# jinlinyi/PerspectiveFields

Measured on AMD Instinct MI355X. Metric: images/sec (640x640, Paramnet-360Cities), higher is better.
Workload: dtype f32 (operands fp32 in HBM; contractions as 2-way fp16 split on the MFMA, fp32 accumulate, fp32-class accuracy); 1 GPU; BASELINE configs[2]: batch 32/GPU 640x640 Paramnet-360Cities-edina-centered, fields + ParamNet, 320x320 network inputs resident in HBM (4 distinct synthetic images tiled over the batch; the network is data independent), post-process to 640x640; global_batch=32, parallelism=dp1 (images sharded, all-gather of ParamNet scalars), weights=seeded synthetic checkpoint (no network for the trained .pth), precision=fp32, tiles=shipped tile table + static heuristic (no tuning), gathered_param_rows=32

## Files before the change

include/pf_hip.h:

```cpp
#ifndef PF_HIP_H
#define PF_HIP_H

#include <stddef.h>
#include <stdint.h>

#ifdef __cplusplus
extern "C" {
#endif

typedef struct pf_engine* pf_handle;

enum pf_status {
  PF_OK = 0,
  PF_ERR_ARG = -1,
  PF_ERR_DEVICE = -2,
  PF_ERR_WEIGHTS = -3,
  PF_ERR_WORKSPACE = -4
};

enum pf_arch {
  PF_ARCH_PARAMNET_CENTERED = 0,
  PF_ARCH_PERSNET_CLS = 1,
  PF_ARCH_PARAMNET_UNCENTERED = 2
};
// ... 79 lines not shown
#define PF_DISPATCH_RB_LAUNCHES 2
#define PF_DISPATCH_SPLITK_LAUNCHES 3
#define PF_DISPATCH_SPLITK_MAX_FACTOR 4
#define PF_DISPATCH_WINO_LAUNCHES 5
#define PF_DISPATCH_WINO_HALF_LAUNCHES 6
#define PF_DISPATCH_THIN128_LAUNCHES 7
#define PF_DISPATCH_ATTN64_LAUNCHES 8
#define PF_DISPATCH_MIT_MLP_FUSED_LAUNCHES 9
#define PF_DISPATCH_LN_KERNEL_LAUNCHES 10
#define PF_DISPATCH_CONV_LAUNCHES 11
#define PF_DISPATCH_SB_TENSORS 12
#define PF_DISPATCH_FORKS 13
#define PF_DISPATCH_FORK_ALLOC_CONFLICTS 14
#define PF_DISPATCH_REAL_PEAK_BYTES 15
#define PF_DISPATCH_DRY_PEAK_BYTES 16
#define PF_DISPATCH_COLS 17
int pf_last_dispatch(pf_handle h, int64_t* out, int n);

int pf_postprocess_batch(pf_handle h, int batch, const float* d_pred_gravity, const float* d_pred_latitude, const int32_t* h_hw,
                         float* const* h_up_out, float* const* h_lat_out, void* d_workspace, size_t workspace_bytes, void* stream);

int pf_fields_from_params(int device, const float* d_cam5, int H, int W, float* d_up, float* d_lat, void* stream);

#define PF_FIT_COL_ROLL 0
#define PF_FIT_COL_PITCH 1
#define PF_FIT_COL_VFOV 2
#define PF_FIT_COL_REL_FOCAL 3
#define PF_FIT_COL_GENERAL_VFOV 4
#define PF_FIT_COL_REL_CX 5
#define PF_FIT_COL_REL_CY 6
#define PF_FIT_COL_RMS_UP 7
// ... 118 lines not shown
```

perspectivefields_amd/build.py:

```python
from __future__ import annotations

import hashlib
import os
import shutil
import subprocess
import sys

HERE = os.path.dirname(os.path.abspath(__file__))
CSRC = os.path.join(HERE, "csrc")
ASAN = os.environ.get("PF_ASAN", "0") == "1"
_VARIANT = ("_tune" if os.environ.get("PF_TUNING_BUILD", "0") == "1" else "") + ("_asan" if ASAN else "") + os.environ.get("PF_LIB_SUFFIX", "")
LIBDIR = os.path.join(HERE, "lib" + _VARIANT)
LIB = os.path.join(LIBDIR, "libpf_hip.so")
SOURCES = ["igemm.hip", "igemm_sb.hip", "igemm_sbf.hip", "igemm_sbh.hip", "wino.hip", "attn.hip", "attn_block.hip", "stem7.hip", "thin_linear.hip", "elem.hip", "dw7.hip", "dw7_pk.hip", "cnx_mlp.hip", "mit_mlp.hip", "rb_gemm.hip", "rb_chain.hip", "fit_camera.hip", "fit_camera_usm.hip", "pano_crop.hip", "field_err.hip", "engine.hip", "engine_ops.hip"]
NO_PK_F32_FLAGS = ["-Xclang", "-target-feature", "-Xclang", "-packed-fp32-ops"]
EXTRA_FLAGS = {"dw7.hip": ["-fno-slp-vectorize"], "dw7_pk.hip": ["-fno-slp-vectorize"],
               "attn_block.hip": NO_PK_F32_FLAGS, "stem7.hip": NO_PK_F32_FLAGS, "thin_linear.hip": NO_PK_F32_FLAGS, "cnx_mlp.hip": NO_PK_F32_FLAGS, "mit_mlp.hip": NO_PK_F32_FLAGS, "rb_gemm.hip": NO_PK_F32_FLAGS, "rb_chain.hip": NO_PK_F32_FLAGS, "fit_camera.hip": NO_PK_F32_FLAGS, "fit_camera_usm.hip": NO_PK_F32_FLAGS, "pano_crop.hip": NO_PK_F32_FLAGS, "field_err.hip": NO_PK_F32_FLAGS}
FLAGS = ["--offload-arch=gfx950", "-O3", "-std=c++17", "-fPIC", "-Wall", "-Wno-unused-function", "-fno-gpu-rdc"]
if os.environ.get("PF_TUNING_BUILD", "0") == "1":
    FLAGS.append("-DPF_TUNING_BUILD")
ASAN_HOST_FLAGS = ["-Xarch_host", "-fsanitize=address,undefined", "-Xarch_host", "-fno-omit-frame-pointer", "-Xarch_host", "-fno-sanitize-recover=undefined"]
if ASAN:
    FLAGS = FLAGS + ASAN_HOST_FLAGS


def asan_runtime() -> str:
    clang = os.path.join(os.path.dirname(os.path.realpath(_hipcc())), "..", "lib", "llvm", "bin", "clang")
    if not os.path.exists(clang):
        clang = "/opt/rocm/lib/llvm/bin/clang"
    return subprocess.run([clang, "-print-file-name=libclang_rt.asan-x86_64.so"], capture_output=True, text=True, check=True).stdout.strip()


# ... 66 lines not shown
```

perspectivefields_amd/csrc/engine.hip:

```cpp
#include <hip/hip_runtime.h>

#include <algorithm>
#include <cmath>
#include <cstdarg>
#include <cstdio>
#include <cstdlib>
#include <cstring>
#include <map>
#include <string>
#include <unordered_map>
#include <vector>

#include "../../include/pf_hip.h"
#include "pf_kernels.h"

using namespace pf;

namespace {

}
namespace pf_host { thread_local std::string g_create_error; }
#include "host_pack.h"
using namespace pf_host;
namespace {
// ... 34 lines not shown
};
struct LNW { float* g = nullptr; float* b = nullptr; int C = 0; float eps = 1e-6f; };
struct DwW { float* w = nullptr; float* b = nullptr; int C = 0; float in_limit = 65504.f;  };

struct RbLin { unsigned short* w = nullptr; size_t bytes = 0; float* inv = nullptr; float* b = nullptr; int N = 0, K = 0; float sat_limit = 65504.f; };
struct RbSrKv { unsigned short* w = nullptr; size_t bytes = 0; float *sr_inv = nullptr, *sr_b = nullptr, *kv_inv = nullptr, *kv_b = nullptr; };
struct RbProjFc1 { unsigned short* w = nullptr; size_t bytes = 0; };
struct MitBlock { LNW n1, n2, srn; RbLin rq, rkv, rproj, rfc1, rfc2; RbSrKv rsrkv; RbProjFc1 rpf; ConvW qln ; ConvW q, kv, proj, sr, fc1, fc2; DwW dw; unsigned short* mlp_w = nullptr; float* mlp_tab = nullptr;
                  unsigned short* a64_w = nullptr; float* a64_tab = nullptr;
                  unsigned short* tq_w = nullptr; float* tq_tab = nullptr; unsigned short* tp_w = nullptr; float* tp_tab = nullptr;  };
struct MitStage { ConvW pe; LNW pen, norm; std::vector<MitBlock> blocks; };
struct Head {
  ConvW lin[4], proc[4], fold[4], r1c1[4], r1c2[4], r2c1[4], r2c2[4], conv0, conv1, predcls;
  float* predw = nullptr; float* predb = nullptr; int nout = 0;
};
struct CnxBlock { float out_limit = 65504.f;  DwW dw; LNW n; ConvW pw1, pw2; unsigned short* mlp_w = nullptr; float* mlp_tab = nullptr;  };
struct Cnx { ConvW stem, ds[3]; LNW stemn, dsn[3], norm; std::vector<CnxBlock> blocks[4]; float* headw = nullptr; float* headb = nullptr; int nout = 0; };

struct SbT {
  unsigned short* p = nullptr;
  size_t plane = 0;
};
struct Ten {
  float* f = nullptr;
  SbT s;
  Ten() {}
  Ten(float* f_) : f(f_) {}
  Ten(float* f_, SbT s_) : f(f_), s(s_) {}
};

struct Profiler;
// ... 207 lines not shown
  int splitk_mode = -1;
  int wino_half = 1;
  bool can_fork(const Ctx& c) { return side_stream_mode && !c.dry && !c.tuning && (!c.prof || c.prof->min_work > 0.0) && side_ready(); }
  bool sba_heads = false;
  int rb_chain = 60;
  int rb_min_blocks = 192;
  int num_cus = 256;
  int wino_min_hw = 20;
  int wino_min_blocks = 96;
  int wino_tile = -1;
  unsigned* d_sat = nullptr;
  float static_window_max = 0.f;
  int mit_mlp128 = 4;
  bool fuse_mit_mlp = true;
  bool fuse_cnx_mlp = true;
  bool fold_mlp = true;
  int nterms = NT_F16X3;
  DebugSink dbg;
  DebugSink* debug_sink = nullptr;
  struct GraphEntry { std::vector<uintptr_t> key; hipGraphExec_t exec; };
  std::vector<GraphEntry> graphs;
  bool sba = false;

  MitStage stages[4];
  ConvW ll;
  Head heads[2];
  Cnx cnx;
  bool has_param = false;
  int param_in = NET;
  float mean3[3] = {103.53f, 116.28f, 123.675f};
// ... 389 lines not shown
          cb.dw = make_dw(b + ".dwconv", C, 7);
          cb.n = make_ln(b + ".norm", C, 1e-6f);
          cb.pw1 = make_linear(b + ".pwconv1", 4 * C, C, nullptr, b + ".norm", 1e-6f);
          const std::vector<float>& gm = get(b + ".gamma", {C}).data;
          std::vector<double> sc(gm.begin(), gm.end());
          cb.pw2 = make_linear(b + ".pwconv2", C, 4 * C, sc.data());
          if (fuse_cnx_mlp && cnx_mlp_preferred(C)) {
            std::vector<unsigned short> wpk;
            std::vector<float> tab;
            cnx_mlp_pack(get(b + ".pwconv1.weight", {4 * C, C}).data.data(), get(b + ".pwconv1.bias", {4 * C}).data.data(), get(b + ".norm.weight", {C}).data.data(),
                         get(b + ".norm.bias", {C}).data.data(), get(b + ".pwconv2.weight", {C, 4 * C}).data.data(), get(b + ".pwconv2.bias", {C}).data.data(), gm.data(), C,
                         &wpk, &tab);
            cb.mlp_w = upload_u16(wpk);
            cb.mlp_tab = upload(tab);
          }
          cnx.blocks[s].push_back(cb);
        }
      }
      for (int s = 0; s < 4; ++s) {
        if (s > 0) cnx.ds[s - 1].sat_limit = cnx.blocks[s][0].dw.in_limit;
        for (size_t j = 0; j < cnx.blocks[s].size(); ++j) {
          const float lim = j + 1 < cnx.blocks[s].size() ? cnx.blocks[s][j + 1].dw.in_limit : 65504.f;
          cnx.blocks[s][j].out_limit = lim;
          cnx.blocks[s][j].pw2.sat_limit = lim;
        }
      }
      note_static(ln_bound(p + "downsample_layers.0.1", CNX_DIMS[0]), cnx.blocks[0][0].dw.in_limit);
      for (int s = 0; s < 4; ++s)
        for (int j = 0; j < CNX_DEPTHS[s]; ++j) {
          const std::string b = p + "stages." + std::to_string(s) + "." + std::to_string(j);
          if (cnx.blocks[s][j].mlp_w) note_static(mlp_hidden_bound(b + ".norm", b + ".pwconv1", "", CNX_DIMS[s]), 65504.f);
        }
      cnx.norm = make_ln(p + "norm", CNX_DIMS[3], 1e-6f);
      cnx.headw = upload(get(p + "head.weight", {cnx.nout, CNX_DIMS[3]}).data);
      cnx.headb = upload(get(p + "head.bias", {cnx.nout}).data);
    }
    for (auto& kv : host)
      if (!kv.second.used) throw fmt("unexpected checkpoint tensor '%s' for this architecture", kv.first.c_str());
    host.clear();
  }

  void tap(Ctx& c, const std::string& name, const float* p, int B, int H, int W, int C) {
    DebugSink* d = c.dbg;
    if (!d || !d->shadow || !p) return;
    const size_t bytes = (size_t)B * H * W * C * 4, off = (d->used + 255) & ~(size_t)255;
    d->taps.push_back({name, off, {B, H, W, C}});
// ... 512 lines not shown
      if (s > 0) {
        const long Mi = (long)B * h * h;
        const Ten yn_in = S ? Ten(nullptr, c.alloc_sb(Mi * CNX_DIMS[s - 1])) : Ten(y);
        ln(c, cnx.dsn[s - 1], y, yn_in, Mi);
        float* yn = c.alloc((size_t)B * (h / 2) * (h / 2) * C);
        conv(c, cnx.ds[s - 1], yn_in, B, h, h, Ten(yn));
        y = yn;
        h /= 2;
      }
      const long M = (long)B * h * h;
      const size_t mk = c.mark();
      float* d = c.alloc(M * C);
      const Ten dn = S ? Ten(nullptr, c.alloc_sb(M * C)) : Ten(d);
      const Ten hb = c.ten(M * 4 * C, !S, S);
      int blk = -1;
      for (CnxBlock& cb : cnx.blocks[s]) {
        if (blk >= 0) tap(c, fmt("pn.s%d.b%d", s + 1, blk), y, B, h, h, C);
        ++blk;
        if (!c.dry) {
          ProfScope ps(c.prof, c.s, PC_DW7, 8.0 * M * C);
          launch_dwconv7x7(y, cb.dw.w, cb.dw.b, d, B, h, h, C, c.s);
        }
        if (cb.mlp_w && nterms == NT_F16X3) {
          range_in(c, fmt("cnx_mlp s%d.b%d d (LN-fused)", s + 1, blk), d, (size_t)M * C);
          if (!c.dry) {
            ProfScope ps(c.prof, c.s, PC_IGEMM_SB, 2.0 * 2.0 * M * (double)C * 4 * C, (int)M, C, 8 * C, 1);
            launch_cnx_mlp(d, y, cb.mlp_w, cb.mlp_tab, M, C, cb.n.eps, c.s, d_sat, cb.out_limit);
          }
          continue;
        }
        if (cb.pw1.ln_s) {
          gemm(c, cb.pw1, Ten(d), M, hb, ACT_GELU);
        } else {
          ln(c, cb.n, d, dn, M);
          gemm(c, cb.pw1, dn, M, hb, ACT_GELU);
        }
        gemm(c, cb.pw2, hb, M, Ten(y), ACT_NONE, y);
      }
      if (blk >= 0) tap(c, fmt("pn.s%d.b%d", s + 1, blk), y, B, h, h, C);
      c.release(mk);
    }
    float* raw = c.alloc((size_t)B * 8);
// ... 172 lines not shown
  if (const char* v = getenv("PF_WINO")) e->wino_min_hw = atoi(v);
  if (const char* v = getenv("PF_WINO_MIN_BLOCKS")) e->wino_min_blocks = atoi(v);
  {
    const char* wt = getenv("PF_WINO_TILE");
    for (int t = 0; t < conv_num_tiles(); ++t) if (strcmp(conv_tile_name(t), wt ? wt : "wino256x64d") == 0) e->wino_tile = t;
  }
  if (const char* v = getenv("PF_RB_CHAIN")) e->rb_chain = atoi(v);
  if (const char* v = getenv("PF_DEFER_AT")) e->defer_at = atoi(v);
  if (const char* v = getenv("PF_DEFER_PRIO")) e->defer_prio = atoi(v);
  if (!host_only) {
    hipDeviceProp_t prop;
    if (hipGetDeviceProperties(&prop, device) == hipSuccess && prop.multiProcessorCount > 0) e->num_cus = prop.multiProcessorCount;
    e->rb_min_blocks = e->num_cus * 3 / 4;
  }
  if (const char* v = getenv("PF_RB_MIN_BLOCKS")) e->rb_min_blocks = atoi(v);
#ifdef PF_TUNING_BUILD
#endif
  if (const char* v = getenv("PF_SIDE_STREAM")) e->side_stream_mode = atoi(v);
  if (const char* v = getenv("PF_S3_SPLIT")) e->s3_split = atoi(v);
  if (const char* v = getenv("PF_ATTN64")) e->attn64 = atoi(v);
  if (const char* v = getenv("PF_STEM7")) e->stem7 = atoi(v);
  if (const char* v = getenv("PF_THIN128")) e->thin128 = atoi(v);
  if (const char* v = getenv("PF_SBA_HEADS")) e->sba_heads = atoi(v) != 0;
  if (const char* v = getenv("PF_AUTOTUNE")) e->autotune = atoi(v) != 0;
  if (const char* v = getenv("PF_SPLIT_BF16")) e->split_bf16 = atoi(v) != 0;
  if (const char* v = getenv("PF_SBA")) e->sba = atoi(v) != 0;
  e->splitk_mode = conv_splitk_env();
  e->wino_half = conv_wino_half_env();
  if (!e->split_bf16) e->sba = false;
  if (!e->split_bf16 || e->sba) e->fuse_ln = false;
  if (!e->split_bf16 || e->sba) e->fuse_cnx_mlp = false;
  if (!e->split_bf16 || e->sba) e->fuse_mit_mlp = false;

  tune_cache_load(e);
  *out = e;
  return PF_OK;
}

int pf_set_precision(pf_handle h, int mode) {
  if (!h) return PF_ERR_ARG;
  if (mode != PF_PRECISION_FP32 && mode != PF_PRECISION_FP32_BF16X6) return h->fail(PF_ERR_ARG, "pf_set_precision: unknown mode (0 = FP32 split-f16, 3 = FP32_BF16X6; the reduced-precision modes 1 / 2 of earlier versions are gone)");
  if (mode != PF_PRECISION_FP32 && !h->split_bf16) return h->fail(PF_ERR_ARG, "pf_set_precision: this mode needs the split kernels (PF_SPLIT_BF16=0 is set)");
  if (h->pn_pending) { h->issue_deferred(); (void)hipStreamSynchronize(h->pstream); h->pn_pending = false; }
  h->ws_cache.clear();
  h->nterms = mode == PF_PRECISION_FP32_BF16X6 ? 6 : NT_F16X3;
  return PF_OK;
}
// ... 649 lines not shown
```

perspectivefields_amd/csrc/engine_ops.hip:

```cpp
#include "host_pack.h"

using namespace pf;
using namespace pf_host;

extern "C" {

int pf_op_num_conv_tiles(void) { return conv_num_tiles(); }
const char* pf_op_conv_tile_name(int id) { return conv_tile_name(id); }

int pf_op_conv2d(int device, const float* x, const float* x2, int B, int H, int W, int C1, int C2, const float* hw, const float* hb,
                 int Cout, int KH, int KW, int stride, int pad, int act, const float* res1, const float* res2, int post_relu,
                 int nchw_out, int tile_id, float* y, const uint16_t* x_planes, long x_plane_elems, const uint16_t* x2_planes,
                 long x2_plane_elems, uint16_t* y_planes, long y_plane_elems, int precision_flags, void* stream) {
  const int precision = precision_flags & 15;
  const bool allow_splitk = !(precision_flags & 16);
  if (precision != PF_PRECISION_FP32 && precision != PF_PRECISION_FP32_BF16X6) { g_create_error = "pf_op_conv2d: precision must be 0 (split-f16) or 3 (exact bf16 split)"; return PF_ERR_ARG; }
  std::string err;
  int rc = check_device(device, &err);
  if (rc != PF_OK) { g_create_error = err; return rc; }
  const int Cin = C1 + C2;
  if (Cin % 4 != 0 || (C2 > 0 && C1 % 32 != 0)) { g_create_error = "pf_op_conv2d: Cin must be a multiple of 4 (pad on the host), C1 of 32 when concatenating"; return PF_ERR_ARG; }
  hipStream_t s = static_cast<hipStream_t>(stream);
  TmpDev tmp;
  ConvParams p;
// ... 331 lines not shown
    float t = 0.f;
    (void)hipEventElapsedTime(&t, a, b);
    *ms_out = t / iters;
    (void)hipEventDestroy(a); (void)hipEventDestroy(b);
  }
  rc = hipGetLastError() == hipSuccess ? PF_OK : PF_ERR_DEVICE;
  tmp.sync_free(s);
  return rc;
}

int pf_op_cnx_mlp(int device, const float* d, float* y, long rows, int C, const float* w1, const float* b1, const float* lng, const float* lnb, float eps,
                  const float* w2, const float* b2, const float* ls, int iters, float* ms_out, void* stream) {
  std::string err;
  int rc = check_device(device, &err);
  if (rc != PF_OK) { g_create_error = err; return rc; }
  if (!cnx_mlp_supported(C) || !d || !y || rows <= 0) { g_create_error = "pf_op_cnx_mlp: C must be 96 or 192"; return PF_ERR_ARG; }
  hipStream_t s = static_cast<hipStream_t>(stream);
  TmpDev tmp;
  std::vector<unsigned short> wpk;
  std::vector<float> tab;
  cnx_mlp_pack(w1, b1, lng, lnb, w2, b2, ls, C, &wpk, &tab);
  const unsigned short* dw = tmp.up_u16(wpk);
  const float* dt = tmp.up(tab);
  launch_cnx_mlp(d, y, dw, dt, rows, C, eps, s);
  if (iters > 0 && ms_out) {
    hipEvent_t a, b;
    (void)hipEventCreate(&a); (void)hipEventCreate(&b);
    (void)hipEventRecord(a, s);
    for (int i = 0; i < iters; ++i) launch_cnx_mlp(d, y, dw, dt, rows, C, eps, s);
    (void)hipEventRecord(b, s);
    (void)hipEventSynchronize(b);
    float t = 0.f;
    (void)hipEventElapsedTime(&t, a, b);
    *ms_out = t / iters;
    (void)hipEventDestroy(a); (void)hipEventDestroy(b);
  }
  rc = hipGetLastError() == hipSuccess ? PF_OK : PF_ERR_DEVICE;
  tmp.sync_free(s);
  return rc;
}

int pf_op_conv2d_bench(int device, int B, int H, int W, int Cin, int Cout, int K, int stride, int pad, int tile_id, int iters, int fmt_prec, float* ms_out) {
  const int fmt = fmt_prec & 15, precision = fmt_prec >> 4;
  std::string err;
// ... 286 lines not shown
```

perspectivefields_amd/csrc/host_pack.h:

```cpp
#pragma once
#include <hip/hip_runtime.h>

#include <algorithm>
#include <cmath>
#include <cstdarg>
#include <cstdio>
#include <cstdlib>
#include <cstring>
#include <string>
#include <vector>

#include "../../include/pf_hip.h"
#include "pf_kernels.h"

namespace pf_host {
using namespace pf;

extern thread_local std::string g_create_error;

inline int roundup(int v, int m) { return (v + m - 1) / m * m; }

inline std::string fmt(const char* f, ...) {
  char buf[1024];
  va_list ap;
// ... 130 lines not shown
  const int npass = N / cols, nct = cols / 32, steps = K / 16;
  const size_t step_us = (size_t)nct * 2 * 512;
  stream->assign(((size_t)npass * steps + 4) * step_us, 0);
  for (int ps = 0; ps < npass; ++ps)
    for (int st = 0; st < steps; ++st) {
      unsigned short* o = stream->data() + ((size_t)ps * steps + st) * step_us;
      for (int ct = 0; ct < nct; ++ct)
        for (int p = 0; p < 2; ++p)
          for (int lane = 0; lane < 64; ++lane)
            for (int e = 0; e < 8; ++e)
              o[((size_t)(ct * 2 + p) * 64 + lane) * 8 + e] = pl.planes[p * n_all + (size_t)(ps * cols + 32 * ct + (lane & 31)) * K + 16 * st + 8 * (lane >> 5) + e];
    }
  *inv = pl.inv_scale;
}

inline void mit_mlp_pack(const float* w1, const float* b1, const float* g, const float* be, const float* wdw , const float* bdw, const float* w2, const float* b2,
                  int C, std::vector<unsigned short>* wpk, std::vector<float>* tab2) {
  const int H = 4 * C, S1 = C / 16, Q = C / 32, NCH = H / 32;
  std::vector<float> w1f, b1f, cs1;
  fold_ln_linear(w1, b1, g, be, H, C, &w1f, &b1f, &cs1);
  std::vector<float> w2v(w2, w2 + (size_t)C * H);
  const F16Planes p1 = split_f16x2(w1f, H), p2 = split_f16x2(w2v, C);
  const size_t n1 = w1f.size(), n2 = w2v.size();
  const size_t chunk_us = (size_t)mit_mlp_chunk_bytes(C) / 2, w1_us = (size_t)S1 * 2 * 512, w2_us = (size_t)Q * 2 * 2 * 512;
  wpk->assign((size_t)NCH * chunk_us, 0);
  for (int t = 0; t < NCH; ++t) {
    unsigned short* o = wpk->data() + (size_t)t * chunk_us;
    for (int s = 0; s < S1; ++s)
      for (int pl = 0; pl < 2; ++pl)
        for (int lane = 0; lane < 64; ++lane)
// ... 57 lines not shown
```

perspectivefields_amd/csrc/pf_kernels.h:

```cpp
#pragma once
#include <vector>
#include <hip/hip_runtime.h>
#include <stddef.h>
#include <stdint.h>

namespace pf {

enum Act { ACT_NONE = 0, ACT_RELU = 1, ACT_GELU = 2 };
#if defined(__HIPCC__)
__device__ __forceinline__ void sat_watch4(unsigned* sat, float limit, float a, float b, float c, float d) {
  const float mx = fmaxf(fmaxf(fabsf(a), fabsf(b)), fmaxf(fabsf(c), fabsf(d)));
  const float s = (a + b) + (c + d);
  if (!(mx <= limit) || s != s) atomicAdd(sat, 1u);
}
__device__ __forceinline__ float sat_acc4(float amax, float a, float b, float c, float d) {
  return __builtin_fmaxf(__builtin_fmaxf(__builtin_fmaxf(amax, __builtin_fabsf(a)), __builtin_fabsf(b)), __builtin_fmaxf(__builtin_fabsf(c), __builtin_fabsf(d)));
}
__device__ __forceinline__ void sat_flush(unsigned* sat, float limit, float amax) {
  if (sat && amax > limit) atomicAdd(sat, 1u);
}
#endif
#if defined(__HIP_DEVICE_COMPILE__)
#define PF_NO_PK_F32 __attribute__((target("no-packed-fp32-ops")))
#else
// ... 189 lines not shown
  int n;
  int H[MAX], W[MAX];
  float rh[MAX], rw[MAX], sxs[MAX], sys[MAX];
  const float* g2[MAX];
  const float* l1[MAX];
  float* up[MAX];
  float* lat[MAX];
};
void launch_postprocess_batch(PostBatch& pb, int h, int w, int lat_is_sin, hipStream_t s);

void launch_nearest_nhwc4(const float* x, float* y, int B, int H, int W, int Ho, int Wo, hipStream_t s);

bool cnx_mlp_supported(int C);
bool cnx_mlp_preferred(int C);
void launch_cnx_mlp(const float* d, float* y, const unsigned short* wpk, const float* tab, long M, int C, float eps, hipStream_t s, unsigned* sat = nullptr, float sat_limit = 65504.f);
bool mit_mlp_supported(int C);
bool mit_mlp_preferred(int C, int with128);
int mit_mlp_chunk_bytes(int C);
void launch_mit_mlp(const float* x, float* y, const unsigned short* wpk, const float* tab2, int B, int Hs, int Ws, int C, float eps, hipStream_t s, unsigned* sat = nullptr, float sat_limit = 65504.f);
struct RbLinArgs {
  const float* x;
  const float* ln_g;
  const float* ln_b;
  float ln_eps;
  const unsigned short* w;
  size_t w_bytes;
  const float* inv;
  const float* bias;
  const float* res;
  float* y;
// ... 115 lines not shown
```

perspectivefields_amd/csrc/rb_common.h:

```cpp
#pragma once
#include "igemm_common.h"
#include "sb_split.h"

namespace pf {

static constexpr int RB_ROWS = 64;
static constexpr int RB_D = 4;

typedef _Float16 rb_f16x8 __attribute__((ext_vector_type(8)));
__device__ __forceinline__ f32x16 rb_mfma(const u32x4 a, const u32x4 b, const f32x16 c) {
  return __builtin_amdgcn_mfma_f32_32x32x16_f16(__builtin_bit_cast(rb_f16x8, a), __builtin_bit_cast(rb_f16x8, b), c, 0, 0, 0);
}

template <int CTW_, bool EXTRA_, int RT_ = 2>
struct RbGeo {
  static constexpr int CTW = CTW_;
  static constexpr bool EXTRA = EXTRA_;
  static constexpr int RT = RT_;
  static constexpr int NW = CTW + (EXTRA ? 1 : 0);
  static constexpr int NACC = RT * CTW + (EXTRA ? 1 : 0);
  static constexpr int NCT = 4 * CTW + (EXTRA ? 2 : 0);
  static constexpr int COLS = NCT * 32;
  static constexpr int STEP_BYTES = NCT * 2048;
  static constexpr int CHS = RT * 2048 + 64;
};

template <class G>
struct RbW {
  __amdgpu_buffer_rsrc_t rw;
  unsigned voff;
  unsigned toff[G::NW];
  u32x4 f[RB_D][G::NW][2];
  __device__ __forceinline__ void init(const unsigned short* w, size_t bytes, int wave, int lane) {
    rw = __builtin_amdgcn_make_buffer_rsrc(const_cast<unsigned short*>(w), 0, (int)(bytes < 0x7fffffffUL ? bytes : 0x7fffffffUL), 0x00020000);
    voff = (unsigned)lane * 16u;
#pragma unroll
    for (int ci = 0; ci < G::NW; ++ci) toff[ci] = (unsigned)__builtin_amdgcn_readfirstlane((ci < G::CTW ? wave + 4 * ci : 4 * G::CTW + (wave >> 1)) * 2048);
  }
  __device__ __forceinline__ void load_frag(int d, int ci, int pl) { f[d][ci][pl] = __builtin_amdgcn_raw_buffer_load_b128(rw, voff + (unsigned)pl * 1024u, toff[ci], 0); }
  __device__ __forceinline__ void advance() { voff += (unsigned)G::STEP_BYTES; }
  __device__ __forceinline__ void load(int d) {
#pragma unroll
    for (int ci = 0; ci < G::NW; ++ci)
#pragma unroll
      for (int pl = 0; pl < 2; ++pl) load_frag(d, ci, pl);
    advance();
  }
  __device__ __forceinline__ void prologue() {
#pragma unroll
    for (int d = 0; d < RB_D; ++d) load(d);
  }
};

template <class G>
struct RbA {
  u32x4 a[G::RT][2];
  u32x4 x[2];
  __device__ __forceinline__ void read(const unsigned char* chunk, int lane, int xr) {
#pragma unroll
    for (int rt = 0; rt < G::RT; ++rt)
#pragma unroll
      for (int pl = 0; pl < 2; ++pl) a[rt][pl] = *reinterpret_cast<const u32x4*>(chunk + (rt * 2 + pl) * 1024 + lane * 16);
    if constexpr (G::EXTRA && G::RT == 2) {
#pragma unroll
      for (int pl = 0; pl < 2; ++pl) x[pl] = *reinterpret_cast<const u32x4*>(chunk + (xr * 2 + pl) * 1024 + lane * 16);
// ... 32 lines not shown
        for (int t = 0; t < 3; ++t)
#pragma unroll
          for (int rt = 0; rt < G::RT; ++rt) acc[G::RT * ci + rt] = rb_mfma(W.f[d][ci][t == 1], A.a[rt][t == 0], acc[G::RT * ci + rt]);
      } else {
#pragma unroll
        for (int t = 0; t < 3; ++t) acc[G::RT * G::CTW] = rb_mfma(W.f[d][ci][t == 1], A.xa(t == 0), acc[G::RT * G::CTW]);
      }
    } else {
      asm volatile("" :: "v"(W.f[d][ci][0]), "v"(W.f[d][ci][1]), "v"(A.a[0][0]), "v"(A.a[G::RT - 1][1]));
    }
    if constexpr ((ABL & 1) == 0) { W.load_frag(d, ci, 0); W.load_frag(d, ci, 1); }
    RB_FENCE();
  }
  W.advance();
}
template <class G, int ABL = 0>
__device__ __forceinline__ void rb_step(f32x16 (&acc)[G::NACC], RbW<G>& W, int d, const RbA<G>& A, RbA<G>& An, const unsigned char* next_chunk, int lane, int xr) {
  if constexpr (ABL != 0) { rb_step_abl<G, ABL>(acc, W, d, A, An, next_chunk, lane, xr); return; }
  constexpr int X = G::CTW, XA = G::RT * G::CTW, RT = G::RT;
  An.read(next_chunk, lane, xr);
  RB_FENCE();
#pragma unroll
  for (int ci = 0; ci < G::CTW; ++ci) {
    const u32x4 (&w)[2] = W.f[d][ci];
#pragma unroll
    for (int rt = 0; rt < RT; ++rt) acc[RT * ci + rt] = rb_mfma(w[0], A.a[rt][1], acc[RT * ci + rt]);
    if (G::EXTRA && ci == 0) {
      acc[XA] = rb_mfma(W.f[d][X][0], A.xa(1), acc[XA]);
      RB_FENCE();
    }
#pragma unroll
    for (int rt = 0; rt < RT; ++rt) acc[RT * ci + rt] = rb_mfma(w[1], A.a[rt][0], acc[RT * ci + rt]);
// ... 40 lines not shown
```

perspectivefields_amd/engine.py:

```python
from __future__ import annotations

import ctypes
import os
from typing import Dict, Optional, Tuple

import numpy as np

from .build import LIB as LIB_PATH

_HERE = os.path.dirname(os.path.abspath(__file__))
TILE_TABLE = os.path.join(_HERE, "tuned", "gfx950_tiles.txt")
NET = 320
PARAMS_STRIDE = 8

PF_OK = 0
DISPATCH_COLUMNS = ("batch", "s3_split_taken", "rb_launches", "splitk_launches", "splitk_max_factor", "wino_launches", "wino_half_launches", "thin128_launches",
                    "attn64_launches", "mit_mlp_fused_launches", "ln_kernel_launches", "conv_launches", "sb_tensors", "forks", "fork_alloc_conflicts",
                    "real_peak_bytes", "dry_peak_bytes")
_STATUS = {0: "PF_OK", -1: "PF_ERR_ARG", -2: "PF_ERR_DEVICE", -3: "PF_ERR_WEIGHTS", -4: "PF_ERR_WORKSPACE"}

_c = ctypes
_P = _c.c_void_p
_SIGNATURES = {
    "pf_version": (_c.c_char_p, []),
    "pf_last_error": (_c.c_char_p, [_P]),
    "pf_create": (_c.c_int, [_c.POINTER(_P), _c.c_int, _c.c_int]),
    "pf_destroy": (_c.c_int, [_P]),
    "pf_load_tensor": (_c.c_int, [_P, _c.c_char_p, _P, _c.POINTER(_c.c_int64), _c.c_int]),
    "pf_finalize_weights": (_c.c_int, [_P]),
    "pf_output_info": (_c.c_int, [_P, _c.POINTER(_c.c_int), _c.POINTER(_c.c_int), _c.POINTER(_c.c_int)]),
    "pf_max_batch": (_c.c_int, []),
    "pf_workspace_bytes": (_c.c_size_t, [_P, _c.c_int]),
    "pf_last_dispatch": (_c.c_int, [_P, _c.POINTER(_c.c_int64), _c.c_int]),
# ... 497 lines not shown
```

Before: 1704 images/sec.

## Fuse ConvNeXt LN+MLP+residual into one row-block kernel for C=384/768

Adds a row-block kernel for ConvNeXt stages 3 and 4 (C=384/768). It fuses LayerNorm, pwconv1, GELU, pwconv2 with layer scale, and the residual add into a single launch. The 4C hidden activation is streamed through LDS in 128-wide chunks instead of being written to HBM, and weights are pre-packed into a fused stream. It is gated by CU-count-based minimum block counts, so small batches fall back to the old path. The cost is a kernel running one block per CU with heavy register and LDS use, and packing complexity.

```diff
diff --git a/include/pf_hip.h b/include/pf_hip.h
--- a/include/pf_hip.h
+++ b/include/pf_hip.h
@@ -117,7 +117,8 @@
 #define PF_DISPATCH_FORK_ALLOC_CONFLICTS 14
 #define PF_DISPATCH_REAL_PEAK_BYTES 15
 #define PF_DISPATCH_DRY_PEAK_BYTES 16
-#define PF_DISPATCH_COLS 17
+#define PF_DISPATCH_CNX_RB_LAUNCHES 17
+#define PF_DISPATCH_COLS 18
 int pf_last_dispatch(pf_handle h, int64_t* out, int n);
 
 int pf_postprocess_batch(pf_handle h, int batch, const float* d_pred_gravity, const float* d_pred_latitude, const int32_t* h_hw,
diff --git a/perspectivefields_amd/build.py b/perspectivefields_amd/build.py
--- a/perspectivefields_amd/build.py
+++ b/perspectivefields_amd/build.py
@@ -12,10 +12,10 @@
 _VARIANT = ("_tune" if os.environ.get("PF_TUNING_BUILD", "0") == "1" else "") + ("_asan" if ASAN else "") + os.environ.get("PF_LIB_SUFFIX", "")
 LIBDIR = os.path.join(HERE, "lib" + _VARIANT)
 LIB = os.path.join(LIBDIR, "libpf_hip.so")
-SOURCES = ["igemm.hip", "igemm_sb.hip", "igemm_sbf.hip", "igemm_sbh.hip", "wino.hip", "attn.hip", "attn_block.hip", "stem7.hip", "thin_linear.hip", "elem.hip", "dw7.hip", "dw7_pk.hip", "cnx_mlp.hip", "mit_mlp.hip", "rb_gemm.hip", "rb_chain.hip", "fit_camera.hip", "fit_camera_usm.hip", "pano_crop.hip", "field_err.hip", "engine.hip", "engine_ops.hip"]
+SOURCES = ["igemm.hip", "igemm_sb.hip", "igemm_sbf.hip", "igemm_sbh.hip", "wino.hip", "attn.hip", "attn_block.hip", "stem7.hip", "thin_linear.hip", "elem.hip", "dw7.hip", "dw7_pk.hip", "cnx_mlp.hip", "mit_mlp.hip", "rb_gemm.hip", "rb_chain.hip", "cnx_rb.hip", "fit_camera.hip", "fit_camera_usm.hip", "pano_crop.hip", "field_err.hip", "engine.hip", "engine_ops.hip"]
 NO_PK_F32_FLAGS = ["-Xclang", "-target-feature", "-Xclang", "-packed-fp32-ops"]
 EXTRA_FLAGS = {"dw7.hip": ["-fno-slp-vectorize"], "dw7_pk.hip": ["-fno-slp-vectorize"],
-               "attn_block.hip": NO_PK_F32_FLAGS, "stem7.hip": NO_PK_F32_FLAGS, "thin_linear.hip": NO_PK_F32_FLAGS, "cnx_mlp.hip": NO_PK_F32_FLAGS, "mit_mlp.hip": NO_PK_F32_FLAGS, "rb_gemm.hip": NO_PK_F32_FLAGS, "rb_chain.hip": NO_PK_F32_FLAGS, "fit_camera.hip": NO_PK_F32_FLAGS, "fit_camera_usm.hip": NO_PK_F32_FLAGS, "pano_crop.hip": NO_PK_F32_FLAGS, "field_err.hip": NO_PK_F32_FLAGS}
+               "attn_block.hip": NO_PK_F32_FLAGS, "stem7.hip": NO_PK_F32_FLAGS, "thin_linear.hip": NO_PK_F32_FLAGS, "cnx_mlp.hip": NO_PK_F32_FLAGS, "mit_mlp.hip": NO_PK_F32_FLAGS, "rb_gemm.hip": NO_PK_F32_FLAGS, "rb_chain.hip": NO_PK_F32_FLAGS, "cnx_rb.hip": NO_PK_F32_FLAGS, "fit_camera.hip": NO_PK_F32_FLAGS, "fit_camera_usm.hip": NO_PK_F32_FLAGS, "pano_crop.hip": NO_PK_F32_FLAGS, "field_err.hip": NO_PK_F32_FLAGS}
 FLAGS = ["--offload-arch=gfx950", "-O3", "-std=c++17", "-fPIC", "-Wall", "-Wno-unused-function", "-fno-gpu-rdc"]
 if os.environ.get("PF_TUNING_BUILD", "0") == "1":
     FLAGS.append("-DPF_TUNING_BUILD")
diff --git a/perspectivefields_amd/csrc/cnx_rb.hip b/perspectivefields_amd/csrc/cnx_rb.hip
--- /dev/null
+++ b/perspectivefields_amd/csrc/cnx_rb.hip
@@ -0,0 +1,205 @@
+#include <stdlib.h>
+
+#include "rb_common.h"
+
+namespace pf {
+
+template <int C>
+__global__ __launch_bounds__(256, 1) void cnx_rb_kernel(const CnxRbArgs p) {
+  static_assert(C == 384 || C == 768, "geometry: 64 x 384 or 32 x 768 row blocks");
+  constexpr int RT = C == 384 ? 2 : 1, ROWS = 32 * RT;
+  using G1 = RbGeo<1, false, RT>;
+  using G2 = RbGeo<C / 128, false, RT>;
+  constexpr int H = 4 * C, HC = G1::COLS, NCH = H / HC, KC = C / 16, KC2 = HC / 16;
+  constexpr int CHS = G1::CHS;
+  constexpr int TPR = 256 / ROWS;
+  constexpr int CPT = KC / TPR;
+  constexpr int TAB = 2 * H + 2 * C, TAB4 = TAB / 4, NTL = (TAB4 + 255) / 256;
+  constexpr int D1 = C == 384 ? 2 * RB_D : RB_D;
+  constexpr unsigned W1_BYTES = KC * G1::STEP_BYTES, W2_BYTES = KC2 * G2::STEP_BYTES;
+  static_assert(HC == 128 && G2::COLS == C && G2::CHS == CHS && KC % TPR == 0 && KC % D1 == 0 && D1 % 2 == 0 && KC2 == 2 * RB_D, "geometry");
+  static_assert(KC2 * CHS >= 4 * 4096, "the epilogue's scratch lives in the A2 region");
+  static_assert(G1::RT == G2::RT && !G1::EXTRA && !G2::EXTRA && sizeof(RbA<G1>) == sizeof(RbA<G2>),
+                "GEMM 2's last look-ahead is handed to GEMM 1 register by register: RbA<G1> and RbA<G2> must be the same fragments");
+  __shared__ __attribute__((aligned(16))) unsigned char As1[KC * CHS];
+  __shared__ __attribute__((aligned(16))) unsigned char As2[KC2 * CHS];
+  __shared__ __attribute__((aligned(16))) float tabs[TAB];
+  const int tid = threadIdx.x, lane = tid & 63, wave = __builtin_amdgcn_readfirstlane(tid >> 6);
+  const int l31 = lane & 31, hi = lane >> 5;
+  const int m0 = blockIdx.x * ROWS;
+  const int nrows = min(ROWS, p.M - m0);
+
+  RbW<G1, D1> W1;
+  RbW<G2> W2;
+  W1.init(p.w, p.w_bytes, wave, lane);
+  W2.init(p.w, p.w_bytes, wave, lane);
+  W2.voff += W1_BYTES;
+
+  {
+    const int r = tid / TPR, q = tid % TPR;
+    const float* xr = p.d + (size_t)(m0 + min(r, nrows - 1)) * C;
+    float4 v[CPT][4];
+#pragma unroll
+    for (int i = 0; i < CPT; ++i)
+#pragma unroll
+      for (int e = 0; e < 4; ++e) v[i][e] = *reinterpret_cast<const float4*>(xr + 16 * (q + TPR * i) + 4 * e);
+    float4 tv[NTL];
+#pragma unroll
+    for (int j = 0; j < NTL; ++j) tv[j] = reinterpret_cast<const float4*>(p.tab)[min(tid + 256 * j, TAB4 - 1)];
+    W1.prologue();
+    float s = 0.f;
+#pragma unroll
+    for (int i = 0; i < CPT; ++i)
+#pragma unroll
+      for (int e = 0; e < 4; ++e) s += (v[i][e].x + v[i][e].y) + (v[i][e].z + v[i][e].w);
+#pragma unroll
+    for (int o = 1; o < TPR; o *= 2) s += __shfl_xor(s, o);
+    const float mu0 = s / (float)C;
+    float s1 = 0.f;
+#pragma unroll
+    for (int i = 0; i < CPT; ++i)
+#pragma unroll
+      for (int e = 0; e < 4; ++e) {
+        v[i][e] = make_float4(v[i][e].x - mu0, v[i][e].y - mu0, v[i][e].z - mu0, v[i][e].w - mu0);
+        s1 += (v[i][e].x + v[i][e].y) + (v[i][e].z + v[i][e].w);
+      }
+#pragma unroll
+    for (int o = 1; o < TPR; o *= 2) s1 += __shfl_xor(s1, o);
+    const float mu = s1 / (float)C;
+    float ss = 0.f;
+#pragma unroll
+    for (int i = 0; i < CPT; ++i)
+#pragma unroll
+      for (int e = 0; e < 4; ++e) {
+        v[i][e] = make_float4(v[i][e].x - mu, v[i][e].y - mu, v[i][e].z - mu, v[i][e].w - mu);
+        ss = fmaf(v[i][e].x, v[i][e].x, fmaf(v[i][e].y, v[i][e].y, fmaf(v[i][e].z, v[i][e].z, fmaf(v[i][e].w, v[i][e].w, ss))));
+      }
+#pragma unroll
+    for (int o = 1; o < TPR; o *= 2) ss += __shfl_xor(ss, o);
+    const float rs = 1.0f / sqrtf(ss * (1.0f / C) + p.ln_eps);
+#pragma unroll
+    for (int i = 0; i < CPT; ++i) {
+#pragma unroll
+      for (int e = 0; e < 4; ++e) {
+        const float4 g = *reinterpret_cast<const float4*>(p.ln_g + 16 * (q + TPR * i) + 4 * e), b = *reinterpret_cast<const float4*>(p.ln_b + 16 * (q + TPR * i) + 4 * e);
+        v[i][e] = make_float4(fmaf(v[i][e].x * rs, g.x, b.x), fmaf(v[i][e].y * rs, g.y, b.y), fmaf(v[i][e].z * rs, g.z, b.z), fmaf(v[i][e].w * rs, g.w, b.w));
+      }
+      rb_store_chunk(As1 + (q + TPR * i) * CHS, r, v[i]);
+    }
+#pragma unroll
+    for (int j = 0; j < NTL; ++j)
+      if (tid + 256 * j < TAB4) reinterpret_cast<float4*>(tabs)[tid + 256 * j] = tv[j];
+  }
+  W2.prologue();
+  __syncthreads();
+
+  f32x16 acc2[G2::NACC];
+#pragma unroll
+  for (int i = 0; i < G2::NACC; ++i)
+#pragma unroll
+    for (int e = 0; e < 16; ++e) acc2[i][e] = 0.f;
+  RbA<G1> A1[2];
+  RbA<G2> A2[2];
+  A1[0].read(As1, lane, 0);
+#pragma unroll 1
+  for (int t = 0; t < NCH; ++t) {
+    f32x16 acc1[G1::NACC];
+#pragma unroll
+    for (int i = 0; i < G1::NACC; ++i)
+#pragma unroll
+      for (int e = 0; e < 16; ++e) acc1[i][e] = 0.f;
+#pragma unroll 1
+    for (int s = 0; s < KC; s += D1) {
+      if (s == KC - D1) W1.voff += W2_BYTES;
+#pragma unroll
+      for (int d = 0; d < D1; ++d) {
+        const int nx = s + d + 1 == KC ? 0 : s + d + 1;
+        rb_step<G1>(acc1, W1, d, A1[d & 1], A1[(d + 1) & 1], As1 + nx * CHS, lane, 0);
+      }
+    }
+    __syncthreads();
+#pragma unroll
+    for (int rt = 0; rt < RT; ++rt)
+#pragma unroll
+      for (int g = 0; g < 4; ++g) {
+        const int n = t * HC + wave * 32 + 8 * g + 4 * hi;
+        const float4 iv = *reinterpret_cast<const float4*>(tabs + n), bb = *reinterpret_cast<const float4*>(tabs + H + n);
+        const float4 hv = make_float4(gelu_erf(fmaf(acc1[rt][4 * g], iv.x, bb.x)), gelu_erf(fmaf(acc1[rt][4 * g + 1], iv.y, bb.y)),
+                                      gelu_erf(fmaf(acc1[rt][4 * g + 2], iv.z, bb.z)), gelu_erf(fmaf(acc1[rt][4 * g + 3], iv.w, bb.w)));
+        uint2 h, l;
+        split4_f16(hv, h, l);
+        unsigned char* dst = As2 + (2 * wave + (g >> 1)) * CHS + rt * 2048 + (l31 + 32 * (g & 1)) * 16 + 8 * hi;
+        *reinterpret_cast<uint2*>(dst) = h;
+        *reinterpret_cast<uint2*>(dst + 1024) = l;
+      }
+    __syncthreads();
+    A2[0].read(As2, lane, 0);
+#pragma unroll
+    for (int s = 0; s < KC2; ++s) {
+      if (s == KC2 - RB_D) W2.voff += W1_BYTES;
+      rb_step<G2>(acc2, W2, s % RB_D, A2[s & 1], A2[(s + 1) & 1], s + 1 < KC2 ? As2 + (s + 1) * CHS : As1, lane, 0);
+    }
+#pragma unroll
+    for (int rt = 0; rt < RT; ++rt)
+#pragma unroll
+      for (int pl = 0; pl < 2; ++pl) A1[0].a[rt][pl] = A2[0].a[rt][pl];
+  }
+  __syncthreads();
+
+  {
+    float* scratch = reinterpret_cast<float*>(As2) + wave * 1024;
+    const float* tinv = tabs + 2 * H;
+    const float* tb = tabs + 2 * H + C;
+    const int rrow = lane >> 3, c4 = lane & 7;
+    float4 rr[G2::NACC][4];
+#pragma unroll
+    for (int idx = 0; idx < G2::NACC; ++idx) {
+      int rt, ct;
+      bool own;
+      rb_tile_of<G2>(idx, wave, rt, ct, own);
+#pragma unroll
+      for (int i = 0; i < 4; ++i) rr[idx][i] = *reinterpret_cast<const float4*>(p.y + (size_t)(m0 + min(rt * 32 + rrow + 8 * i, nrows - 1)) * C + ct * 32 + c4 * 4);
+    }
+#pragma unroll
+    for (int idx = 0; idx < G2::NACC; ++idx) {
+      int rt, ct;
+      bool own;
+      rb_tile_of<G2>(idx, wave, rt, ct, own);
+#pragma unroll
+      for (int g = 0; g < 4; ++g)
+        *reinterpret_cast<float4*>(scratch + l31 * 32 + (((2 * g + hi) ^ (l31 & 7)) << 2)) = make_float4(acc2[idx][4 * g], acc2[idx][4 * g + 1], acc2[idx][4 * g + 2], acc2[idx][4 * g + 3]);
+      __builtin_amdgcn_wave_barrier();
+      const int n = ct * 32 + c4 * 4;
+      const float4 iv = *reinterpret_cast<const float4*>(tinv + n), bb = *reinterpret_cast<const float4*>(tb + n);
+      float4 v[4];
+#pragma unroll
+      for (int i = 0; i < 4; ++i) {
+        const int row = rrow + 8 * i;
+        v[i] = *reinterpret_cast<const float4*>(scratch + row * 32 + ((c4 ^ (row & 7)) << 2));
+      }
+      __builtin_amdgcn_wave_barrier();
+#pragma unroll
+      for (int i = 0; i < 4; ++i) {
+        const int ml = rt * 32 + rrow + 8 * i;
+        const float4 w = make_float4(fmaf(v[i].x, iv.x, bb.x) + rr[idx][i].x, fmaf(v[i].y, iv.y, bb.y) + rr[idx][i].y, fmaf(v[i].z, iv.z, bb.z) + rr[idx][i].z,
+                                     fmaf(v[i].w, iv.w, bb.w) + rr[idx][i].w);
+        if (own && ml < nrows) {
+          if (p.sat) sat_watch4(p.sat, p.sat_limit, w.x, w.y, w.z, w.w);
+          *reinterpret_cast<float4*>(p.y + (size_t)(m0 + ml) * C + n) = w;
+        }
+      }
+    }
+  }
+}
+
+bool cnx_rb_supported(int C) { return C == 384 || C == 768; }
+int cnx_rb_rows(int C) { return C == 384 ? 64 : 32; }
+
+void launch_cnx_rb(const CnxRbArgs& a, int C, hipStream_t s) {
+  const int rows = cnx_rb_rows(C);
+  const dim3 grid((unsigned)((a.M + rows - 1) / rows)), block(256);
+  if (C == 384) hipLaunchKernelGGL((cnx_rb_kernel<384>), grid, block, 0, s, a);
+  else if (C == 768) hipLaunchKernelGGL((cnx_rb_kernel<768>), grid, block, 0, s, a);
+}
+
+}
diff --git a/perspectivefields_amd/csrc/engine.hip b/perspectivefields_amd/csrc/engine.hip
--- a/perspectivefields_amd/csrc/engine.hip
+++ b/perspectivefields_amd/csrc/engine.hip
@@ -72,7 +72,8 @@
   ConvW lin[4], proc[4], fold[4], r1c1[4], r1c2[4], r2c1[4], r2c2[4], conv0, conv1, predcls;
   float* predw = nullptr; float* predb = nullptr; int nout = 0;
 };
-struct CnxBlock { float out_limit = 65504.f;  DwW dw; LNW n; ConvW pw1, pw2; unsigned short* mlp_w = nullptr; float* mlp_tab = nullptr;  };
+struct CnxBlock { float out_limit = 65504.f;  DwW dw; LNW n; ConvW pw1, pw2; unsigned short* mlp_w = nullptr; float* mlp_tab = nullptr;
+                  unsigned short* rb_w = nullptr; size_t rb_w_bytes = 0; float* rb_tab = nullptr;  };
 struct Cnx { ConvW stem, ds[3]; LNW stemn, dsn[3], norm; std::vector<CnxBlock> blocks[4]; float* headw = nullptr; float* headb = nullptr; int nout = 0; };
 
 struct SbT {
@@ -310,6 +311,8 @@
   int mit_mlp128 = 4;
   bool fuse_mit_mlp = true;
   bool fuse_cnx_mlp = true;
+  int cnx_rb = 1;
+  int cnx_rb_min_blocks[2] = {96, 192};
   bool fold_mlp = true;
   int nterms = NT_F16X3;
   DebugSink dbg;
@@ -729,6 +732,15 @@
             cb.mlp_w = upload_u16(wpk);
             cb.mlp_tab = upload(tab);
           }
+          if ((cnx_rb & 3) && cnx_rb_supported(C) && !((cnx_rb & 4) && C != 384)) {
+            std::vector<unsigned short> wpk;
+            std::vector<float> tab;
+            cnx_rb_pack(get(b + ".pwconv1.weight", {4 * C, C}).data.data(), get(b + ".pwconv1.bias", {4 * C}).data.data(), get(b + ".pwconv2.weight", {C, 4 * C}).data.data(),
+                        get(b + ".pwconv2.bias", {C}).data.data(), gm.data(), C, &wpk, &tab);
+            cb.rb_w = upload_u16(wpk);
+            cb.rb_w_bytes = wpk.size() * 2;
+            cb.rb_tab = upload(tab);
+          }
           cnx.blocks[s].push_back(cb);
         }
       }
@@ -744,7 +756,7 @@
       for (int s = 0; s < 4; ++s)
         for (int j = 0; j < CNX_DEPTHS[s]; ++j) {
           const std::string b = p + "stages." + std::to_string(s) + "." + std::to_string(j);
-          if (cnx.blocks[s][j].mlp_w) note_static(mlp_hidden_bound(b + ".norm", b + ".pwconv1", "", CNX_DIMS[s]), 65504.f);
+          if (cnx.blocks[s][j].mlp_w || cnx.blocks[s][j].rb_w) note_static(mlp_hidden_bound(b + ".norm", b + ".pwconv1", "", CNX_DIMS[s]), 65504.f);
         }
       cnx.norm = make_ln(p + "norm", CNX_DIMS[3], 1e-6f);
       cnx.headw = upload(get(p + "head.weight", {cnx.nout, CNX_DIMS[3]}).data);
@@ -1287,6 +1299,8 @@
       const Ten dn = S ? Ten(nullptr, c.alloc_sb(M * C)) : Ten(d);
       const Ten hb = c.ten(M * 4 * C, !S, S);
       int blk = -1;
+      const long cnx_rb_blocks = cnx_rb_supported(C) ? (M + cnx_rb_rows(C) - 1) / cnx_rb_rows(C) : 0;
+      const bool use_cnx_rb = (cnx_rb & 3) && nterms == NT_F16X3 && !S && !c.tuning && cnx_rb_blocks > 0 && ((cnx_rb & 3) == 2 || cnx_rb_blocks >= cnx_rb_min_blocks[C == 384 ? 0 : 1]);
       for (CnxBlock& cb : cnx.blocks[s]) {
         if (blk >= 0) tap(c, fmt("pn.s%d.b%d", s + 1, blk), y, B, h, h, C);
         ++blk;
@@ -1299,6 +1313,18 @@
           if (!c.dry) {
             ProfScope ps(c.prof, c.s, PC_IGEMM_SB, 2.0 * 2.0 * M * (double)C * 4 * C, (int)M, C, 8 * C, 1);
             launch_cnx_mlp(d, y, cb.mlp_w, cb.mlp_tab, M, C, cb.n.eps, c.s, d_sat, cb.out_limit);
+          }
+          continue;
+        }
+        if (cb.rb_w && use_cnx_rb) {
+          range_in(c, fmt("cnx_rb s%d.b%d d (LN input)", s + 1, blk), d, (size_t)M * C);
+          if (!c.dry) {
+            CnxRbArgs a;
+            a.d = d; a.y = y; a.w = cb.rb_w; a.w_bytes = cb.rb_w_bytes; a.tab = cb.rb_tab; a.ln_g = cb.n.g; a.ln_b = cb.n.b; a.ln_eps = cb.n.eps; a.M = (int)M;
+            a.sat = d_sat; a.sat_limit = cb.out_limit;
+            ProfScope ps(c.prof, c.s, PC_IGEMM_SB, 2.0 * 2.0 * M * (double)C * 4 * C, (int)M, C, 8 * C, 1);
+            c.count(PF_DISPATCH_CNX_RB_LAUNCHES);
+            launch_cnx_rb(a, C, c.s);
           }
           continue;
         }
@@ -1501,6 +1527,10 @@
     e->rb_min_blocks = e->num_cus * 3 / 4;
   }
   if (const char* v = getenv("PF_RB_MIN_BLOCKS")) e->rb_min_blocks = atoi(v);
+  if (const char* v = getenv("PF_CNX_RB")) e->cnx_rb = atoi(v);
+  if (!host_only) { e->cnx_rb_min_blocks[0] = e->num_cus * 3 / 8; e->cnx_rb_min_blocks[1] = e->num_cus * 3 / 4; }
+  if (const char* v = getenv("PF_CNX_RB_MIN_BLOCKS")) e->cnx_rb_min_blocks[0] = atoi(v);
+  if (const char* v = getenv("PF_CNX_RB_MIN_BLOCKS_768")) e->cnx_rb_min_blocks[1] = atoi(v);
 #ifdef PF_TUNING_BUILD
 #endif
   if (const char* v = getenv("PF_SIDE_STREAM")) e->side_stream_mode = atoi(v);
@@ -1518,6 +1548,7 @@
   if (!e->split_bf16 || e->sba) e->fuse_ln = false;
   if (!e->split_bf16 || e->sba) e->fuse_cnx_mlp = false;
   if (!e->split_bf16 || e->sba) e->fuse_mit_mlp = false;
+  if (!e->split_bf16 || e->sba) e->cnx_rb = 0;
 
   tune_cache_load(e);
   *out = e;
diff --git a/perspectivefields_amd/csrc/engine_ops.hip b/perspectivefields_amd/csrc/engine_ops.hip
--- a/perspectivefields_amd/csrc/engine_ops.hip
+++ b/perspectivefields_amd/csrc/engine_ops.hip
@@ -369,20 +369,29 @@
   std::string err;
   int rc = check_device(device, &err);
   if (rc != PF_OK) { g_create_error = err; return rc; }
-  if (!cnx_mlp_supported(C) || !d || !y || rows <= 0) { g_create_error = "pf_op_cnx_mlp: C must be 96 or 192"; return PF_ERR_ARG; }
+  if ((!cnx_mlp_supported(C) && !cnx_rb_supported(C)) || !d || !y || rows <= 0 || rows > 0x7fffffffL / (4 * C)) { g_create_error = "pf_op_cnx_mlp: C must be 96, 192, 384 or 768"; return PF_ERR_ARG; }
   hipStream_t s = static_cast<hipStream_t>(stream);
   TmpDev tmp;
   std::vector<unsigned short> wpk;
   std::vector<float> tab;
-  cnx_mlp_pack(w1, b1, lng, lnb, w2, b2, ls, C, &wpk, &tab);
+  const bool rb = cnx_rb_supported(C);
+  if (rb) cnx_rb_pack(w1, b1, w2, b2, ls, C, &wpk, &tab);
+  else cnx_mlp_pack(w1, b1, lng, lnb, w2, b2, ls, C, &wpk, &tab);
   const unsigned short* dw = tmp.up_u16(wpk);
   const float* dt = tmp.up(tab);
-  launch_cnx_mlp(d, y, dw, dt, rows, C, eps, s);
+  CnxRbArgs ra{};
+  if (rb) {
+    ra.d = d; ra.y = y; ra.w = dw; ra.w_bytes = wpk.size() * 2; ra.tab = dt; ra.ln_g = tmp.up(lng, C); ra.ln_b = tmp.up(lnb, C); ra.ln_eps = eps; ra.M = (int)rows;
+    ra.sat = nullptr; ra.sat_limit = 65504.f;
+    if (!dw || !dt || !ra.ln_g || !ra.ln_b) { g_create_error = "pf_op_cnx_mlp: hipMalloc failed"; tmp.sync_free(s); return PF_ERR_DEVICE; }
+  }
+  auto launch = [&]() { if (rb) launch_cnx_rb(ra, C, s); else launch_cnx_mlp(d, y, dw, dt, rows, C, eps, s); };
+  launch();
   if (iters > 0 && ms_out) {
     hipEvent_t a, b;
     (void)hipEventCreate(&a); (void)hipEventCreate(&b);
     (void)hipEventRecord(a, s);
-    for (int i = 0; i < iters; ++i) launch_cnx_mlp(d, y, dw, dt, rows, C, eps, s);
+    for (int i = 0; i < iters; ++i) launch();
     (void)hipEventRecord(b, s);
     (void)hipEventSynchronize(b);
     float t = 0.f;
diff --git a/perspectivefields_amd/csrc/host_pack.h b/perspectivefields_amd/csrc/host_pack.h
--- a/perspectivefields_amd/csrc/host_pack.h
+++ b/perspectivefields_amd/csrc/host_pack.h
@@ -168,6 +168,38 @@
   *inv = pl.inv_scale;
 }
 
+inline void cnx_rb_pack(const float* w1, const float* b1, const float* w2, const float* b2, const float* ls, int C, std::vector<unsigned short>* stream, std::vector<float>* tab) {
+  const int H = 4 * C, HC = 128, NCH = H / HC, KC = C / 16, KC2 = HC / 16, NCT2 = C / 32;
+  std::vector<float> w1v(w1, w1 + (size_t)H * C), w2f((size_t)C * H), b2f(C);
+  for (int n = 0; n < C; ++n) {
+    for (int j = 0; j < H; ++j) w2f[(size_t)n * H + j] = (float)((double)w2[(size_t)n * H + j] * (double)ls[n]);
+    b2f[n] = (float)((double)b2[n] * (double)ls[n]);
+  }
+  const F16Planes p1 = split_f16x2(w1v, H), p2 = split_f16x2(w2f, C);
+  const size_t n1 = w1v.size(), n2 = w2f.size();
+  const size_t step1 = (size_t)4 * 2 * 512, step2 = (size_t)NCT2 * 2 * 512, chunk = KC * step1 + KC2 * step2;
+  stream->assign((size_t)NCH * chunk + KC * step1 + 4 * step2, 0);
+  for (int t = 0; t < NCH; ++t) {
+    unsigned short* o = stream->data() + (size_t)t * chunk;
+    for (int st = 0; st < KC; ++st)
+      for (int ct = 0; ct < 4; ++ct)
+        for (int p = 0; p < 2; ++p)
+          for (int lane = 0; lane < 64; ++lane)
+            for (int e = 0; e < 8; ++e)
+              o[st * step1 + ((size_t)(ct * 2 + p) * 64 + lane) * 8 + e] = p1.planes[p * n1 + (size_t)(HC * t + 32 * ct + (lane & 31)) * C + 16 * st + 8 * (lane >> 5) + e];
+    o += KC * step1;
+    for (int st = 0; st < KC2; ++st)
+      for (int ct = 0; ct < NCT2; ++ct)
+        for (int p = 0; p < 2; ++p)
+          for (int lane = 0; lane < 64; ++lane)
+            for (int e = 0; e < 8; ++e)
+              o[st * step2 + ((size_t)(ct * 2 + p) * 64 + lane) * 8 + e] = p2.planes[p * n2 + (size_t)(32 * ct + (lane & 31)) * H + HC * t + 16 * st + 8 * (lane >> 5) + e];
+  }
+  tab->resize((size_t)2 * H + 2 * C);
+  for (int j = 0; j < H; ++j) { (*tab)[j] = p1.inv_scale[j]; (*tab)[H + j] = b1[j]; }
+  for (int n = 0; n < C; ++n) { (*tab)[2 * H + n] = p2.inv_scale[n]; (*tab)[2 * H + C + n] = b2f[n]; }
+}
+
 inline void mit_mlp_pack(const float* w1, const float* b1, const float* g, const float* be, const float* wdw , const float* bdw, const float* w2, const float* b2,
                   int C, std::vector<unsigned short>* wpk, std::vector<float>* tab2) {
   const int H = 4 * C, S1 = C / 16, Q = C / 32, NCH = H / 32;
diff --git a/perspectivefields_amd/csrc/pf_kernels.h b/perspectivefields_amd/csrc/pf_kernels.h
--- a/perspectivefields_amd/csrc/pf_kernels.h
+++ b/perspectivefields_amd/csrc/pf_kernels.h
@@ -227,6 +227,22 @@
 bool cnx_mlp_supported(int C);
 bool cnx_mlp_preferred(int C);
 void launch_cnx_mlp(const float* d, float* y, const unsigned short* wpk, const float* tab, long M, int C, float eps, hipStream_t s, unsigned* sat = nullptr, float sat_limit = 65504.f);
+struct CnxRbArgs {
+  const float* d;
+  float* y;
+  const unsigned short* w;
+  size_t w_bytes;
+  const float* tab;
+  const float* ln_g;
+  const float* ln_b;
+  float ln_eps;
+  int M;
+  unsigned* sat = nullptr;
+  float sat_limit = 65504.f;
+};
+bool cnx_rb_supported(int C);
+int cnx_rb_rows(int C);
+void launch_cnx_rb(const CnxRbArgs& a, int C, hipStream_t s);
 bool mit_mlp_supported(int C);
 bool mit_mlp_preferred(int C, int with128);
 int mit_mlp_chunk_bytes(int C);
diff --git a/perspectivefields_amd/csrc/rb_common.h b/perspectivefields_amd/csrc/rb_common.h
--- a/perspectivefields_amd/csrc/rb_common.h
+++ b/perspectivefields_amd/csrc/rb_common.h
@@ -25,12 +25,12 @@
   static constexpr int CHS = RT * 2048 + 64;
 };
 
-template <class G>
+template <class G, int D = RB_D>
 struct RbW {
   __amdgpu_buffer_rsrc_t rw;
   unsigned voff;
   unsigned toff[G::NW];
-  u32x4 f[RB_D][G::NW][2];
+  u32x4 f[D][G::NW][2];
   __device__ __forceinline__ void init(const unsigned short* w, size_t bytes, int wave, int lane) {
     rw = __builtin_amdgcn_make_buffer_rsrc(const_cast<unsigned short*>(w), 0, (int)(bytes < 0x7fffffffUL ? bytes : 0x7fffffffUL), 0x00020000);
     voff = (unsigned)lane * 16u;
@@ -48,7 +48,7 @@
   }
   __device__ __forceinline__ void prologue() {
 #pragma unroll
-    for (int d = 0; d < RB_D; ++d) load(d);
+    for (int d = 0; d < D; ++d) load(d);
   }
 };
 
@@ -111,8 +111,8 @@
   }
   W.advance();
 }
-template <class G, int ABL = 0>
-__device__ __forceinline__ void rb_step(f32x16 (&acc)[G::NACC], RbW<G>& W, int d, const RbA<G>& A, RbA<G>& An, const unsigned char* next_chunk, int lane, int xr) {
+template <class G, int ABL = 0, int D = RB_D>
+__device__ __forceinline__ void rb_step(f32x16 (&acc)[G::NACC], RbW<G, D>& W, int d, const RbA<G>& A, RbA<G>& An, const unsigned char* next_chunk, int lane, int xr) {
   if constexpr (ABL != 0) { rb_step_abl<G, ABL>(acc, W, d, A, An, next_chunk, lane, xr); return; }
   constexpr int X = G::CTW, XA = G::RT * G::CTW, RT = G::RT;
   An.read(next_chunk, lane, xr);
diff --git a/perspectivefields_amd/engine.py b/perspectivefields_amd/engine.py
--- a/perspectivefields_amd/engine.py
+++ b/perspectivefields_amd/engine.py
@@ -16,7 +16,7 @@
 PF_OK = 0
 DISPATCH_COLUMNS = ("batch", "s3_split_taken", "rb_launches", "splitk_launches", "splitk_max_factor", "wino_launches", "wino_half_launches", "thin128_launches",
                     "attn64_launches", "mit_mlp_fused_launches", "ln_kernel_launches", "conv_launches", "sb_tensors", "forks", "fork_alloc_conflicts",
-                    "real_peak_bytes", "dry_peak_bytes")
+                    "real_peak_bytes", "dry_peak_bytes", "cnx_rb_launches")
 _STATUS = {0: "PF_OK", -1: "PF_ERR_ARG", -2: "PF_ERR_DEVICE", -3: "PF_ERR_WEIGHTS", -4: "PF_ERR_WORKSPACE"}
 
 _c = ctypes
```

Result: faster. 1736 images/sec (median of 6 runs) (+1.9%).
